# calad0i/da4ml

Hardware: AMD Instinct MI355X
Metric: CMVM solves/sec, 256x256 int8 matrix (higher is better)
Workload: dtype u32; 1 GPU; c3_256x256_int8_batch64_single_chain; matrix=256x256 int8 (default_rng(seed).integers(-128,128)), batch_per_gpu=64, parallelism=1 x independent-instance shard, no data-path collective

## Files before the change

### __graft_entry__.py

```python

import subprocess
import sys
from pathlib import Path

ROOT = Path(__file__).resolve().parent
if str(ROOT) not in sys.path:
    sys.path.insert(0, str(ROOT))


def build() -> None:
    subprocess.run(['make', '-C', str(ROOT / 'da4ml_amd' / 'csrc')], check=True)
    subprocess.run(['make', '-C', str(ROOT / 'oracle'), 'liboracle.so', 'ref'], check=True)
    subprocess.run(['make', '-C', str(ROOT / 'tests' / 'model')], check=True)
    subprocess.run(['make', '-C', str(ROOT / 'tests' / 'geometry')], check=True)
    subprocess.run(['make', '-C', str(ROOT / 'tests' / 'emu')], check=True)
    import da4ml_amd
    from da4ml_amd import _binary

    lib = _binary.lib()
    missing = [s for s in _binary.EXPORTS if not hasattr(lib, s)]
    assert not missing, f'libda4ml_hip.so lacks {missing}'


def smoke() -> None:
    import numpy as np

    from da4ml_amd import _binary
    from oracle.oracle import Oracle

    assert _binary.device_count() >= 1, 'smoke() needs a HIP device'
    k = np.random.default_rng(0).integers(-8, 8, (16, 16)).astype(np.float32)
    got = _binary.solve(k, adder_size=1, carry_size=-1)
    want = Oracle('port').solve(k, adder_size=1, carry_size=-1)
    assert got == want, 'HIP solve differs from the CPU oracle'
    assert np.all(got.kernel == k)
    print(f'smoke ok: 16x16 int4 cost={got.cost} adders={got.n_adders} latency={got.latency}')


if __name__ == '__main__':
    build()
    if len(sys.argv) > 1 and sys.argv[1] == 'smoke':
        smoke()
```

### da4ml_amd/csrc/cmvm_core.h

```cpp
#pragma once

#include <stdint.h>
#include <string.h>

#if defined(__HIPCC__)
#include <hip/hip_runtime.h>
#define DA_HD __host__ __device__ __forceinline__
#else
#define DA_HD inline
#endif

namespace da {

enum Method : int { M_MC = 0, M_MC_DC = 1, M_MC_PDC = 2, M_WMC = 3, M_WMC_DC = 4, M_WMC_PDC = 5, M_DUMMY = 6 };

enum ChainError : int {
    E_OK = 0,
    E_ROW_CAPACITY = 1,
    E_TABLE_CAPACITY = 2,
    E_LIST_CAPACITY = 3,
    E_FLOAT_DOMAIN = 4,
    E_COUNT_OVERFLOW = 5,
    E_REMOTE_ERROR = 6,
};

struct RowInfo {
    float lo, hi, step, lat;
};

DA_HD uint32_t f2u(float f) {
    uint32_t u;
    memcpy(&u, &f, 4);
    return u;
}
DA_HD float u2f(uint32_t u) {
    float f;
    memcpy(&f, &u, 4);
    return f;
}
DA_HD int popc32(uint32_t x) {
#if defined(__HIP_DEVICE_COMPILE__)
    return __popc(x);
#else
    return __builtin_popcount(x);
#endif
}
DA_HD int ctz32(uint32_t x) {
#if defined(__HIP_DEVICE_COMPILE__)
    return __ffs((int)x) - 1;
#else
    return __builtin_ctz(x);
#endif
}

template <class Cell> struct CellOps;
template <> struct CellOps<uint32_t> {
    static constexpr int HALF = 16;
    static DA_HD uint32_t plus(uint32_t c) { return c & 0xFFFFu; }
    static DA_HD uint32_t minus(uint32_t c) { return c >> 16; }
    static DA_HD uint32_t make(uint32_t p, uint32_t m) { return p | (m << 16); }
};
template <> struct CellOps<uint64_t> {
    static constexpr int HALF = 32;
    static DA_HD uint32_t plus(uint64_t c) { return (uint32_t)c; }
    static DA_HD uint32_t minus(uint64_t c) { return (uint32_t)(c >> 32); }
    static DA_HD uint64_t make(uint32_t p, uint32_t m) { return (uint64_t)p | ((uint64_t)m << 32); }
};

DA_HD int key_count(int n_bits) { return 2 * (2 * n_bits - 1); }
DA_HD int key_index(int shift, int sub, int n_bits) { return sub * (2 * n_bits - 1) + shift + (n_bits - 1); }
DA_HD void key_decode(int idx, int n_bits, int &shift, int &sub) {
    int w = 2 * n_bits - 1;
    sub = idx >= w;
    shift = idx - sub * w - (n_bits - 1);
}

DA_HD uint32_t take_from(uint32_t x, int s) { return s >= 0 ? (s >= 32 ? 0u : x >> s) : (-s >= 32 ? 0u : x << (-s)); }
DA_HD uint32_t move_by(uint32_t x, int s) { return take_from(x, -s); }

DA_HD void naf_masks(int32_t x, uint32_t &plus, uint32_t &minus) {
    uint32_t a = x < 0 ? (uint32_t)(-(int64_t)x) : (uint32_t)x;
    uint64_t x3 = (uint64_t)a * 3u;
    uint32_t pos = (uint32_t)((x3 & ~(uint64_t)a) >> 1);
    uint32_t neg = (uint32_t)((~x3 & (uint64_t)a) >> 1);
    plus = x < 0 ? neg : pos;
    minus = x < 0 ? pos : neg;
}
DA_HD int naf_weight(int32_t x) {
    uint32_t a = x < 0 ? (uint32_t)(-(int64_t)x) : (uint32_t)x;
    uint64_t x3 = (uint64_t)a * 3u;
    uint64_t d = (x3 ^ (uint64_t)a) >> 1;
    return popc32((uint32_t)d) + popc32((uint32_t)(d >> 32));
}
DA_HD int csd_width(uint32_t max_abs) {
    uint64_t t = 3ull * (max_abs ? max_abs : 1u);
    int n = 1;
    while ((1ull << (n + 1)) < t) ++n;
    return n;
}
DA_HD int lsb_loc(float x) {
    if (x == 0.0f) return 127;
    uint32_t b = f2u(x);
    int e = (int)((b >> 23) & 0xFF);
    uint32_t m = (b & 0x7FFFFFu) + (1u << 23);
    return (int)(int8_t)(e + ctz32(m) - 150);
}
DA_HD int iceil_log2(float x) {
    uint32_t b = f2u(x);
    int e = (int)((b >> 23) & 0xFF);
    return (int)(int8_t)(e - 127 + ((b & 0x7FFFFFu) != 0));
}
DA_HD float pow2f(int s) { return u2f((uint32_t)(s + 127) << 23); }

template <class Cell, class F> DA_HD void for_pairs_cross(Cell lo, Cell hi, int n_bits, F &&f) {
    using O = CellOps<Cell>;
    uint32_t lp = O::plus(lo), lm = O::minus(lo), hp = O::plus(hi), hm = O::minus(hi);
    uint32_t la = lp | lm, ha = hp | hm;
    while (la) {
        int p = ctz32(la);
        la &= la - 1;
        int sl = (lm >> p) & 1;
        uint32_t h = ha;
        while (h) {
            int q = ctz32(h);
            h &= h - 1;
            int sh = (hm >> q) & 1;
            f(key_index(q - p, sl ^ sh, n_bits));
        }
    }
}
template <class Cell, class F> DA_HD void for_pairs_self(Cell c, int n_bits, F &&f) {
    using O = CellOps<Cell>;
    uint32_t cp = O::plus(c), cm = O::minus(c);
    uint32_t all = cp | cm;
    uint32_t hi = all;
    while (hi) {
        int a = ctz32(hi);
        hi &= hi - 1;
        int sa = (cm >> a) & 1;
        uint32_t lo = all & ((1u << a) - 1u);
        while (lo) {
            int b = ctz32(lo);
            lo &= lo - 1;
            int sb = (cm >> b) & 1;
            f(key_index(b - a, sa ^ sb, n_bits));
        }
    }
}
template <class Cell, class F> DA_HD void for_pairs_part(Cell part, Cell y, bool x_is_lo, int n_bits, F &&f) {
    if (x_is_lo)
        for_pairs_cross<Cell>(part, y, n_bits, f);
    else
        for_pairs_cross<Cell>(y, part, n_bits, f);
}

template <class Cell> DA_HD void substitute_column(Cell a, Cell b, bool same_row, int shift, int sub, Cell &ma, Cell &mb) {
    using O = CellOps<Cell>;
    uint32_t ap = O::plus(a), am = O::minus(a);
    if (!same_row) {
        uint32_t bp = O::plus(b), bm = O::minus(b);
        uint32_t map = ap & take_from(sub ? bm : bp, shift);
        uint32_t mam = am & take_from(sub ? bp : bm, shift);
        uint32_t tp = move_by(map, shift), tm = move_by(mam, shift);
        ma = O::make(map, mam);
        mb = sub ? O::make(tm, tp) : O::make(tp, tm);
        return;
    }
    int rel = -shift;
    uint32_t avp = ap, avm = am, map = 0, mam = 0, mbp = 0, mbm = 0;
    for (int p = 0; p + rel < O::HALF; ++p) {
        uint32_t bit_lo = 1u << p, bit_hi = 1u << (p + rel);
        uint32_t all = avp | avm;
        if (!(all & bit_lo) || !(all & bit_hi)) continue;
        int s_lo = (avm & bit_lo) != 0, s_hi = (avm & bit_hi) != 0;
        if ((s_lo ^ s_hi) != sub) continue;
        avp &= ~(bit_lo | bit_hi);
        avm &= ~(bit_lo | bit_hi);
        if (s_hi)
            mam |= bit_hi;
        else
            map |= bit_hi;
        if (s_lo)
            mbm |= bit_lo;
        else
            mbp |= bit_lo;
    }
    ma = O::make(map, mam);
    mb = O::make(mbp, mbm);
}

DA_HD int n_overlap(const RowInfo &a, const RowInfo &b) {
    float hi0 = a.hi + a.step, hi1 = b.hi + b.step;
    float st = a.step > b.step ? a.step : b.step;
    int8_t f = (int8_t)(-iceil_log2(st));
    float m0 = __builtin_fabsf(a.lo) < __builtin_fabsf(hi0) ? __builtin_fabsf(hi0) : __builtin_fabsf(a.lo);
    float m1 = __builtin_fabsf(b.lo) < __builtin_fabsf(hi1) ? __builtin_fabsf(hi1) : __builtin_fabsf(b.lo);
    int8_t i_low = (int8_t)iceil_log2(m1 < m0 ? m1 : m0);
    int8_t k = (a.lo < 0 || b.lo < 0) ? 1 : 0;
    return (int)(int8_t)(k + i_low + f);
}

DA_HD uint32_t float_rank(float s) {
    if (s != s) return 0;
    if (s == 0.0f) s = 0.0f;
    uint32_t u = f2u(s == 0.0f ? 0.0f : s);
    return (u & 0x80000000u) ? ~u : (u | 0x80000000u);
}

DA_HD uint32_t entry_rank(uint32_t count, int ov, float dl, int method) {
    if (count < 2) return 0;
    switch (method) {
    case M_MC: return count + 1;
    case M_WMC: {
#if defined(__HIP_DEVICE_COMPILE__)
        if (count <= 0xFFFFu) {
            const int32_t s32 = (int32_t)count * ov;
            return s32 >= 0 ? (uint32_t)s32 + 1 : 0;
        }
#endif
        int64_t s = (int64_t)count * ov;
        return s >= 0 ? (uint32_t)s + 1 : 0;
    }
    case M_MC_DC:
    case M_MC_PDC: {
#if defined(__HIP_DEVICE_COMPILE__)
        float s = __fsub_rn((float)count, __fmul_rn(1e9f, dl));
#else
// ... 136 lines not shown
```

### da4ml_amd/csrc/cmvm_engine.hip

```cpp

#include <hip/hip_runtime.h>

#include <algorithm>
#include <atomic>
#include <chrono>
#include <cmath>
#include <cstdio>
#include <cstdlib>
#include <cstring>
#include <memory>
#include <mutex>
#include <numeric>
#include <stdexcept>
#include <string>
#include <thread>
#include <vector>

#include "cmvm_core.h"
#include "cmvm_geometry.h"
#include "cmvm_gpu.h"
#include "cmvm_host.h"

namespace da {
namespace gpu {
// ... 1927 lines not shown
            }
        }
        (void)w;
    }
    if (c.rword && part == 1) {
        const int nl = (int)gq->l_n[(gq->iter - 1) & 1];
        const CandEntry *ll = &gq->l_list[(gq->iter - 1) & 1][0];
        const uint32_t *colbits = gq->colbits;
        const int cbw = gq->cb_words;
        for (int e = (wave_id() + 2) % UPD_WAVES; e < nl; e += UPD_WAVES) {
            const unsigned long long tw = ll[e].tie;
            const uint32_t i0 = (uint32_t)((tw >> 7) & 0xFFFFFFu), i1 = (uint32_t)(tw >> 31);
            const uint32_t r = (i0 == A || i0 == B) ? i1 : i0;
            int hit = 0;
            for (int k = lane; k < u.m; k += WAVE) hit |= (int)((colbits[(size_t)u.mcol[k] * cbw + (r >> 5)] >> (r & 31)) & 1u);
            if (!__any(hit) && lane == 0) fold_entry(c, (uint32_t)ll[e].rank, tw);
        }
    }
}

template <class Cell, int NWV, bool STATS>
__device__ __forceinline__ void update_body(ChainDev *gq, bool in_range, int block_y, int grid_y) {
    constexpr int NTHR = NWV * WAVE;
    const UpdStep<Cell> u = load_upd_step<Cell>(gq);
    if (!in_range || u.done) return;
    if (block_y >= grid_y - 2) {
        special_pairs<Cell>(gq, u, block_y - (grid_y - 2));
        return;
    }
    grid_y -= 2;
    if (block_y * (NWV * QN) >= u.n_partners) return;
    extern __shared__ __attribute__((aligned(16))) unsigned char smem[];
    const int tid = threadIdx.x, lane = lane_id(), wid = wave_id();
    UpdLds<Cell> s;
    s.carve(smem, smem + align16(UpdLds<Cell>::table_bytes(u.c.n_out)) + (size_t)wid * UpdLds<Cell>::wave_bytes(u.c.Kpad), u.c.n_out);
    const int total_waves = grid_y * NWV, gw = block_y * NWV + wid;
    const unsigned long long ref0 = gw * QN + (lane >> QG_LOG2) < u.n_partners ? u.plist[gw * QN + (lane >> QG_LOG2)] : 0ull;
    const RowInfo rnew = load_row(u.c.rows, u.Nw);
    __shared__ unsigned int s_stat[3];
    if constexpr (STATS)
        if (tid < 3) s_stat[tid] = 0;
    copy_handoff<Cell>(u, s, tid, NTHR);
    __syncthreads();
    unsigned int found = 0, inserts = 0, deletes = 0;
    update_partners<Cell, STATS>(gq, u, s, gw * QN, total_waves * QN, u.n_partners, ref0, rnew, found, inserts, deletes);
    if constexpr (!STATS) return;
    if (lane == 0 && (found | inserts | deletes)) {
        if (found) atomicAdd(&s_stat[0], found);
        if (inserts) atomicAdd(&s_stat[1], inserts);
        if (deletes) atomicAdd(&s_stat[2], deletes);
    }
    __syncthreads();
    if (tid == 0) {
        if (s_stat[0]) atomicAdd(&gq->st_found, (unsigned long long)s_stat[0]);
        if (s_stat[1]) atomicAdd(&gq->st_inserts, (unsigned long long)s_stat[1]);
        if (s_stat[1] != s_stat[2]) atomicAdd(&gq->n_live, s_stat[1] - s_stat[2]);
    }
}
template <class Cell, bool STATS>
__global__ void __launch_bounds__(UPD_THREADS, DA_UPD_OCC) __attribute__((amdgpu_num_sgpr(DA_UPD_SGPRS))) k_iter_update(ChainDev *chains, int n_chains) {
#ifdef DA_STEP_CLOCKS
    ChainDev *gk = &chains[(int)blockIdx.x < n_chains ? blockIdx.x : 0];
    const bool clk_on = (int)blockIdx.x < n_chains && !gk->done;
    const int clk_par = (gk->iter - 1) & 1;
    if (clk_on && threadIdx.x == 0) CLK_MARK(gk, clk_par, 2, true);
#endif
    update_body<Cell, UPD_WAVES, STATS>(&chains[(int)blockIdx.x < n_chains ? blockIdx.x : 0], (int)blockIdx.x < n_chains, (int)blockIdx.y, (int)gridDim.y);
#ifdef DA_STEP_CLOCKS
    __syncthreads();
    if (clk_on && threadIdx.x == 0) CLK_MARK(gk, clk_par, 3, false);
#endif
}


template <class Cell> __global__ void __launch_bounds__(256) k_cs_init_counts(ChainDev *g) {
    const Ctx c = make_ctx(g, 0);
    extern __shared__ __attribute__((aligned(16))) unsigned char smem[];
    uint32_t *cnt = reinterpret_cast<uint32_t *>(smem) + (size_t)wave_id() * c.Kpad;
    const long long n_in = g->n_in, n_pairs = n_in * (n_in + 1) / 2;
    const long long p = (long long)blockIdx.x * (blockDim.x / WAVE) + wave_id();
    if (p >= n_pairs) return;
    long long i1 = (long long)((sqrt(8.0 * (double)p + 1.0) - 1.0) * 0.5);
    while (i1 * (i1 + 1) / 2 > p) --i1;
    while ((i1 + 1) * (i1 + 2) / 2 <= p) ++i1;
    const uint32_t hi = (uint32_t)i1, lo = (uint32_t)(p - i1 * (i1 + 1) / 2);
    count_row_pair<Cell>(c, reinterpret_cast<const typename RowFmt<Cell>::Entry *>(g->rlist), lo, hi, cnt);
    for (int k = lane_id(); k < c.K; k += WAVE) g->cs_init[(size_t)p * c.K + k] = (int32_t)cnt[k];
}
template <class Cell> __global__ void __launch_bounds__(256) k_cs_init_table(ChainDev *g) {
    const Ctx c = make_ctx(g, 0);
    const long long n_in = g->n_in, n_pairs = n_in * (n_in + 1) / 2;
    const long long p = (long long)blockIdx.x * (blockDim.x / WAVE) + wave_id();
    if (p >= n_pairs) return;
    long long i1 = (long long)((sqrt(8.0 * (double)p + 1.0) - 1.0) * 0.5);
    while (i1 * (i1 + 1) / 2 > p) --i1;
    while ((i1 + 1) * (i1 + 2) / 2 <= p) ++i1;
    const uint32_t hi = (uint32_t)i1, lo = (uint32_t)(p - i1 * (i1 + 1) / 2);
    const int32_t *cnt = g->cs_init + (size_t)p * c.K;
    int f = 0;
    for (int k = lane_id(); k < c.K; k += WAVE) f |= cnt[k] >= 2;
    if (!__any(f)) return;
    if (c.method < 0) {
        if (lane_id() == 0) g->unknown_hit = 1;
        return;
    }
    table_insert(c, lo, hi, load_row(c.rows, lo), load_row(c.rows, hi), [&](int k) { return (uint32_t)cnt[k]; });
}

__global__ void __launch_bounds__(1024) k_cs_union(ChainDev *g, volatile int *report, int seq, int flag_words) {
    __shared__ int s_part[16], s_base[17];
    const int tid = threadIdx.x, lane = lane_id(), wid = wave_id();
    const int n_rows = (int)g->Nw;
    const int per = (n_rows + 1023) / 1024;
    const int r0 = min(tid * per, n_rows), r1 = min(r0 + per, n_rows);
    int mine = 0;
    for (int r = r0; r < r1; ++r) mine += ((g->cs_flags[r >> 2] >> (8 * (r & 3))) & 0xFF) != 0;
    int inc = mine;
    for (int o = 1; o < WAVE; o <<= 1) {
        int t = __shfl_up(inc, o);
        if (lane >= o) inc += t;
    }
    if (lane == WAVE - 1) s_part[wid] = inc;
    __syncthreads();
    if (tid == 0) {
        int run = 0;
        for (int w = 0; w < 16; ++w) {
            s_base[w] = run;
            run += s_part[w];
        }
        s_base[16] = run;
        g->cs_nuni = run;
        if (report) {
            report[1] = run;
            report[2] = g->cs_flags[flag_words];
            report[3] = g->cs_flags[flag_words + 1];
            report[4] = g->cs_flags[flag_words + 2];
            __threadfence_system();
            report[0] = seq;
        }
    }
    __syncthreads();
    int at = s_base[wid] + inc - mine;
    for (int r = r0; r < r1; ++r)
        if (((g->cs_flags[r >> 2] >> (8 * (r & 3))) & 0xFF) != 0) g->cs_uni[at++] = (uint32_t)r;
}

template <class Cell> __global__ void __launch_bounds__(256) k_cs_partial(ChainDev *g) {
    using F = RowFmt<Cell>;
    using Entry = typename F::Entry;
    const Ctx c = make_ctx(g, 0);
    const int m = g->m, nb = c.n_bits, n_out = c.n_out, K = c.K, Kpad = c.Kpad;
    extern __shared__ __attribute__((aligned(16))) unsigned char smem[];
    Cell *s_mA = reinterpret_cast<Cell *>(smem);
    Cell *s_mB = s_mA + n_out;
    uint32_t *s_cnt = reinterpret_cast<uint32_t *>(s_mB + n_out);
    uint16_t *s_cmap = reinterpret_cast<uint16_t *>(s_cnt + 4 * 3 * Kpad);
    const int tid = threadIdx.x, lane = lane_id(), wid = wave_id();
    for (int j = tid; j < n_out; j += 256) s_cmap[j] = 0;
    __syncthreads();
    for (int j = tid; j < m; j += 256) {
        s_cmap[g->mcol[j]] = (uint16_t)(j + 1);
        s_mA[j] = reinterpret_cast<const Cell *>(g->mA)[j];
        s_mB[j] = reinterpret_cast<const Cell *>(g->mB)[j];
    }
    __syncthreads();
    const int u = (int)blockIdx.x * 4 + wid;
    if (u >= g->cs_nuni) return;
    const uint32_t A = g->A, B = g->B, r = g->cs_uni[u];
    const bool same = A == B;
    uint32_t *dA = s_cnt + (size_t)wid * 3 * Kpad, *dB = dA + Kpad, *cN = dB + Kpad;
    for (int k = lane; k < 3 * Kpad; k += WAVE) dA[k] = 0;
    lds_fence();
    const da_u2 ref = g->rowoff[r];
    const Entry *row = reinterpret_cast<const Entry *>(g->rlist) + ref.x;
    for (int j = lane; j < (int)ref.y; j += WAVE) {
        const Entry en = row[j];
        const Cell x = F::cell(en);
        if (!x) continue;
        const int at = (int)s_cmap[F::col(en)];
        if (!at) continue;
        const Cell ma = s_mA[at - 1], mb = s_mB[at - 1];
        for_pairs_part<Cell>(ma, x, A < r, nb, [&](int k) { atomicAdd(&dA[k], 1u); });
        if (same)
            for_pairs_part<Cell>(mb, x, A < r, nb, [&](int k) { atomicAdd(&dA[k], 1u); });
        else
            for_pairs_part<Cell>(mb, x, B < r, nb, [&](int k) { atomicAdd(&dB[k], 1u); });
        for_pairs_cross<Cell>(x, ma, nb, [&](int k) { atomicAdd(&cN[k], 1u); });
    }
    lds_fence();
    int32_t *out = g->cs_slab + (size_t)(6 + 3 * u) * K;
    for (int k = lane; k < K; k += WAVE) {
        out[k] = (int32_t)dA[k];
        out[K + k] = (int32_t)dB[k];
        out[2 * K + k] = (int32_t)cN[k];
    }
}

template <class Cell> __global__ void __launch_bounds__(256) k_cs_apply(ChainDev *g) {
    Ctx c = make_ctx(g, 2 * g->iter - 1);
    c.rword = g->spec[(g->iter - 1) & 1].word;
    c.cn = &g->c_n[(g->iter - 1) & 1];
    c.cl = &g->c_list[(g->iter - 1) & 1][0];
    const int K = c.K;
    const int w = (int)blockIdx.x * 4 + wave_id();
    const uint32_t A = g->A, B = g->B, Nw = g->Nw;
    const bool same = A == B;
    if (w == 5 && c.rword) {
        const int nl = (int)g->l_n[(g->iter - 1) & 1];
        const CandEntry *ll = &g->l_list[(g->iter - 1) & 1][0];
        if (lane_id() == 0)
            for (int e = 0; e < nl; ++e) {
                const unsigned long long tw = ll[e].tie;
                const uint32_t i0 = (uint32_t)((tw >> 7) & 0xFFFFFFu), i1 = (uint32_t)(tw >> 31);
                const uint32_t r = (i0 == A || i0 == B) ? i1 : i0;
                if (((g->cs_flags[r >> 2] >> (8 * (r & 3))) & 0xFF) == 0) fold_entry(c, (uint32_t)ll[e].rank, tw);
            }
    }
    if (w < 6) {
        uint32_t lo = A, hi = A;
        bool active = true, existed = false;
        switch (w) {
        case 0: lo = A, hi = A, existed = true; break;
        case 1: lo = A, hi = B, existed = true, active = !same; break;
        case 2: lo = B, hi = B, existed = true, active = !same; break;
        case 3: lo = A, hi = Nw; break;
        case 4: lo = B, hi = Nw, active = !same; break;
        default: lo = Nw, hi = Nw; break;
        }
        if (!active) return;
        const int32_t *cnt = g->cs_slab + (size_t)w * K;
        const unsigned long long key = pack_pair(lo, hi);
        const int slot = existed ? table_find(c, key, hash_pair(lo, hi)) : -1;
        if (slot >= 0)
            table_update(c, slot, key, [&](int k, uint32_t) { return (uint32_t)cnt[k]; });
        else {
            int f = 0;
            for (int k = lane_id(); k < K; k += WAVE) f |= cnt[k] >= 2;
            if (__any(f)) table_insert(c, lo, hi, load_row(c.rows, lo), load_row(c.rows, hi), [&](int k) { return (uint32_t)cnt[k]; });
        }
        return;
    }
    const int u = w - 6;
    if (u >= g->cs_nuni) return;
    const uint32_t r = g->cs_uni[u];
    const int32_t *dA = g->cs_slab + (size_t)(6 + 3 * u) * K, *dB = dA + K, *cN = dB + K;
    {
        const uint32_t lo = min(A, r), hi = max(A, r);
        const int slot = table_find(c, pack_pair(lo, hi), hash_pair(lo, hi));
        if (slot >= 0) table_update(c, slot, pack_pair(lo, hi), [&](int k, uint32_t old) { return old - (uint32_t)dA[k]; });
    }
    if (!same) {
        const uint32_t lo = min(B, r), hi = max(B, r);
        const int slot = table_find(c, pack_pair(lo, hi), hash_pair(lo, hi));
        if (slot >= 0) table_update(c, slot, pack_pair(lo, hi), [&](int k, uint32_t old) { return old - (uint32_t)dB[k]; });
    }
    int f = 0;
    for (int k = lane_id(); k < K; k += WAVE) f |= cN[k] >= 2;
    if (__any(f)) table_insert(c, r, Nw, load_row(c.rows, r), load_row(c.rows, Nw), [&](int k) { return (uint32_t)cN[k]; });
    if (lane_id() == 0) atomicAdd(&g->st_partners, 1ull);
}

template <class Cell> __global__ void __launch_bounds__(256) k_extract(ChainDev *chains) {
    using O = CellOps<Cell>;
    using F = RowFmt<Cell>;
    ChainDev &ch = chains[blockIdx.y];
    int j = blockIdx.x * (blockDim.x / WAVE) + wave_id();
    if (j >= ch.n_out) return;
    const auto *rl = reinterpret_cast<const typename F::Entry *>(ch.rlist);
    int lane = lane_id(), len = ch.collen[j], out = 0;
    for (int base = 0; base < len; base += WAVE) {
        int e = base + lane;
        Cell c = 0;
        uint32_t r = 0;
        if (e < len) {
            const unsigned long long ref = ch.collist[(size_t)j * ch.lcap + e];
            r = ref_row(ref);
            const auto *row = rl + ref_off(ref);
            if ((int)r < ch.n_in)
                c = F::cell(row[j]);
            else {
                int lo = 0, hi = (int)ref_len(ref) - 1;
                while (lo < hi) {
                    int mid = (lo + hi) >> 1;
                    if (F::col(row[mid]) < (uint32_t)j)
                        lo = mid + 1;
                    else
                        hi = mid;
                }
                const auto en = row[lo];
                c = F::col(en) == (uint32_t)j ? F::cell(en) : (Cell)0;
            }
        }
        unsigned long long nz = __ballot(c != 0);
        if (c != 0) {
            size_t at = (size_t)j * ch.lcap + out + __popcll(nz & ((1ull << lane) - 1));
            ch.fin_row[at] = r;
            ch.fin_cell[at] = (unsigned long long)O::plus(c) | ((unsigned long long)O::minus(c) << 32);
        }
        out += __popcll(nz);
    }
    if (lane == 0) ch.fin_count[j] = (uint32_t)out;
}

__global__ void __launch_bounds__(256) k_pack(ChainDev *chains) {
    ChainDev &ch = chains[blockIdx.x];
    __shared__ uint32_t s_total;
    const int n_out = ch.n_out, tid = threadIdx.x, lane = lane_id(), nw = blockDim.x / WAVE;
    if (tid < WAVE) {
        uint32_t run = 0;
        for (int base = 0; base < n_out; base += WAVE) {
            int j = base + lane;
            uint32_t v = j < n_out ? ch.fin_count[j] : 0u, inc = v;
            for (int o = 1; o < WAVE; o <<= 1) {
                uint32_t t = (uint32_t)__shfl_up((int)inc, o);
                if (lane >= o) inc += t;
            }
            if (j < n_out) ch.fin_start[j] = run + inc - v;
            run += (uint32_t)__shfl((int)inc, WAVE - 1);
        }
        if (lane == 0) {
            ch.fin_start[n_out] = run;
            ch.pk_total = run;
            s_total = run;
        }
    }
    __syncthreads();
    if (s_total > (uint32_t)ch.pk_cap) {
        if (tid == 0) ch.error = E_LIST_CAPACITY;
        return;
    }
    for (int j = wave_id(); j < n_out; j += nw) {
        const uint32_t cnt = ch.fin_count[j], dst = ch.fin_start[j];
        const size_t src = (size_t)j * ch.lcap;
        for (uint32_t e = lane; e < cnt; e += WAVE) {
            ch.pk_row[dst + e] = ch.fin_row[src + e];
            ch.pk_cell[dst + e] = ch.fin_cell[src + e];
        }
    }
    for (int r = tid; r < ch.n_rows; r += blockDim.x) ch.pk_lat[r] = ch.rows[r].lat;
}

struct GatherPiece {
    const void *src;
    unsigned long long dst_off, bytes;
};
__global__ void __launch_bounds__(256) k_gather(const GatherPiece *pieces, unsigned char *dst) {
// ... 782 lines not shown
        o.stats.digits0 = d.prep_digits;
        o.stats.table_peak = d.live_peak;
        o.stats.scan_slots = (long long)d.st_rescans << d.gs_log2;
        o.stats.partners = (long long)d.st_partners;
        o.stats.matches = (long long)d.st_matches;
        for (int q = 0; q < 12; ++q) im.timings.phase_cycles[q] += (double)d.st_phase[q];
        for (int q = 0; q < 4; ++q) im.timings.search_cycles[q] += (double)d.st_qphase[q];
        im.timings.search_diag[0] += (double)d.st_qdiag[0], im.timings.search_diag[1] += (double)d.st_qdiag[1], im.timings.search_diag[2] += (double)d.st_qdiag[4];
        im.timings.search_diag[3] += (double)d.st_qdiag[5], im.timings.search_diag[4] = std::max(im.timings.search_diag[4], (double)d.st_qdiag[6]), im.timings.search_diag[5] += (double)d.st_qdiag[7], im.timings.search_diag[6] += (double)d.st_qdiag[8];
        im.timings.fast_steps += (long long)d.st_fast;
        im.timings.found += (long long)d.st_found;
        im.timings.inserts += (long long)d.st_inserts;
        im.timings.cell_reads += (long long)d.st_cells;
        im.timings.key_bytes += 2.0 * d.K * (double)(d.st_found + d.st_inserts);
        im.timings.cell_bytes += (geo[i].wide ? 8.0 : 4.0) * (double)d.st_cells;
        im.timings.iterations += d.iter;
        im.timings.rescans += (long long)d.st_rescans;
        im.timings.select_bytes += (double)d.st_sel_bytes + 32.0 * (double)d.n_groups * (double)d.iter + (double)d.st_rescans * ((double)(4u << d.gs_log2) + 24.0);
        im.timings.partners += (long long)d.st_partners;
        im.timings.table_bytes += (double)d.C * (8.0 + 4.0 + (double)(1 << d.pb_log2));
    }
    lap("extract + download + unpack");
    im.timings.loop_ms += loop_ms;
    im.timings.host_launch_ms += host_launch_ms;
    im.timings.lockstep_iters += launched_iters;
    im.timings.chains += n;
    im.timings.arena_bytes = std::max(im.timings.arena_bytes, (double)arena_bytes);
    im.timings.total_ms += std::chrono::duration<double, std::milli>(std::chrono::steady_clock::now() - t_begin).count();
    (void)max_n_in;
}

namespace {

class HipShardEngine : public ShardEngine {
  public:
    HipShardEngine(hipStream_t st, int device, const ChainJob &job, int c0, int c1, double table_scale, double row_scale)
        : st_(st), device_(device), job_(job), n_loc_(c1 - c0) {
        HIP_CHECK(hipSetDevice(device_));
        const size_t e = (size_t)job.n_in * job.n_out;
        const size_t kb = align_up(e * 4, 256), qb = align_up((size_t)job.n_in * 12, 256), lb = align_up((size_t)job.n_in * 4, 256);
        io_.get(2 * kb + qb + lb + align_up(job.n_in, 256) + align_up(job.n_out, 256) + 256);
        unsigned char *io = static_cast<unsigned char *>(io_.ptr);
        std::memset(&d_, 0, sizeof d_);
        d_.n_in = job.n_in;
        d_.n_out = n_loc_;
        d_.pn_out = job.n_out;
        d_.col0 = c0;
        d_.method = job.method;
        d_.adder_size = job.adder_size;
        d_.carry_size = job.carry_size;
        d_.kernel = reinterpret_cast<const float *>(io);
        d_.qints = reinterpret_cast<const float *>(io + kb);
        d_.lats = reinterpret_cast<const float *>(io + kb + qb);
        d_.xint = reinterpret_cast<int32_t *>(io + kb + qb + lb);
        d_.shift0 = reinterpret_cast<int8_t *>(io + 2 * kb + qb + lb);
        d_.shift1 = d_.shift0 + align_up(job.n_in, 256);
        HIP_CHECK(hipMemcpyAsync(io, job.kernel, e * 4, hipMemcpyHostToDevice, st_));
        HIP_CHECK(hipMemcpyAsync(io + kb, job.qints, (size_t)job.n_in * 12, hipMemcpyHostToDevice, st_));
        HIP_CHECK(hipMemcpyAsync(io + kb + qb, job.lats, (size_t)job.n_in * 4, hipMemcpyHostToDevice, st_));
        desc_.get(sizeof(ChainDev));
        dd_ = static_cast<ChainDev *>(desc_.ptr);
        push();
        hipLaunchKernelGGL(k_prepare, dim3(1), dim3(256), (size_t)job.n_out * 4, st_, dd_);
        HIP_CHECK(hipGetLastError());
        pull();
        Geometry &g = geo_;
        g.n_bits = d_.prep_nbits;
        if (g.n_bits > 30) throw std::runtime_error("kernel needs more than 30 CSD digits per entry; unsupported");
        g.wide = g.n_bits > 12 || n_loc_ > 256;
        if (job.adder_size >= 0 || job.carry_size >= 0) step_tab_.build(job.qints, job.n_in);
        g.n_mant = (int)step_tab_.mant.size();
        g.K = key_count(g.n_bits);
        g.Kpad = (g.K + 3) & ~3;
        g.pb_log2 = 5;
        while ((1 << g.pb_log2) < 16 + 2 * g.Kpad) ++g.pb_log2;
        const long long D0 = d_.prep_digits;
        const TableGeometry tg = table_geometry(job, d_.prep_pairs, D0, table_scale, row_scale, MAX_GROUPS);
        g.rcap = tg.rcap < (1 << REF_ROW_BITS) ? (int)tg.rcap : (1 << REF_ROW_BITS);
        g.lcap = job.n_in + d_.prep_maxdcol + 1;
        g.pk_cap = (int)std::min<long long>(D0 + 1, (long long)1 << 30);
        const long long rl_want = (long long)job.n_in * n_loc_ + D0 + n_loc_ + 64;
        if (rl_want >= (1ll << REF_OFF_BITS) || g.rcap >= (1 << REF_ROW_BITS) || n_loc_ >= (1 << REF_LEN_BITS))
            throw std::runtime_error("problem too large for the row-reference format");
        g.rl_cap = (uint32_t)rl_want;
        g.C = tg.C;
        g.gs_log2 = tg.gs_log2;
        g.n_groups = tg.n_groups;
        n_pairs_ = (long long)job.n_in * (job.n_in + 1) / 2;
        ChainJob local = job;
        local.n_out = n_loc_;
        ChainDev tmp;
        const size_t chain_bytes = carve_chain(nullptr, local, g, tmp);
        const size_t init_b = align_up((size_t)n_pairs_ * g.K * 4, 256), flag_b = align_up((((size_t)g.rcap + 3) / 4 + SHARD_TRAILER) * 4 + 64, 256),
                     uni_b = align_up((size_t)g.rcap * 4, 256), slab_b = align_up((size_t)(6 + 3 * (size_t)g.rcap) * g.K * 4, 256);
        const size_t need = chain_bytes + init_b + flag_b + uni_b + slab_b;
        {
            size_t free_b = 0, total_b = 0;
            HIP_CHECK(hipMemGetInfo(&free_b, &total_b));
            if (need > free_b)
                throw std::runtime_error("a column-sharded chain needs " + std::to_string(need >> 20) + " MiB of device memory (pair table of " +
                                         std::to_string(g.C) + " slots), " + std::to_string(free_b >> 20) + " MiB are free");
        }
        arena_.get(need);
        unsigned char *a = static_cast<unsigned char *>(arena_.ptr);
        carve_chain(a, local, g, d_);
        d_.cs_init = reinterpret_cast<int32_t *>(a + chain_bytes);
        d_.cs_flags = reinterpret_cast<int32_t *>(a + chain_bytes + init_b);
        d_.cs_uni = reinterpret_cast<uint32_t *>(a + chain_bytes + init_b + flag_b);
        d_.cs_slab = reinterpret_cast<int32_t *>(a + chain_bytes + init_b + flag_b + uni_b);
        d_.n_bits = g.n_bits;
        d_.K = g.K;
        d_.Kpad = g.Kpad;
        d_.rcap = g.rcap;
        d_.lcap = g.lcap;
        d_.gs_log2 = g.gs_log2;
        d_.n_groups = g.n_groups;
        d_.C = g.C;
        d_.cmask = g.C - 1;
        d_.pb_log2 = g.pb_log2;
        d_.rl_cap = g.rl_cap;
        d_.rl_used = (uint32_t)job.n_in * (uint32_t)n_loc_;
        d_.n_rows = job.n_in;
        d_.claim_words = claim_words_for(local_job(), g, sel2_lds_budget(device_, g.wide));
        HIP_CHECK(hipMemsetAsync(d_.stamp, 0, sizeof(uint32_t) * (size_t)g.rcap, st_));
        HIP_CHECK(hipMemsetAsync(d_.hkey, 0xFF, sizeof(unsigned long long) * (size_t)g.C, st_));
        HIP_CHECK(hipMemsetAsync(d_.hrank, 0, sizeof(uint32_t) * (size_t)g.C, st_));
        HIP_CHECK(hipMemsetAsync(d_.grec, 0, sizeof(GroupRec) * (size_t)g.n_groups, st_));
        d_.cb_words = (g.rcap + 31) / 32;
        HIP_CHECK(hipMemsetAsync(d_.colbits, 0, sizeof(uint32_t) * (size_t)n_loc_ * d_.cb_words, st_));
        {
            d_.n_step_mant = (int)step_tab_.mant.size();
            if (d_.n_step_mant) {
                HIP_CHECK(hipMemcpyAsync(const_cast<uint32_t *>(d_.step_mant), step_tab_.mant.data(), step_tab_.mant.size() * 4, hipMemcpyHostToDevice, st_));
                HIP_CHECK(hipMemcpyAsync(const_cast<float *>(d_.step_tab), step_tab_.tab.data(), step_tab_.tab.size() * 4, hipMemcpyHostToDevice, st_));
            }
        }
        push();
        report_ = static_cast<volatile int *>(report_buf_.get(64));
        for (int q = 0; q < 5; ++q) report_[q] = 0;
        d_done_ = static_cast<unsigned int *>(done_buf_.get(sizeof(unsigned int)));
        HIP_CHECK(hipMemsetAsync(d_done_, 0, sizeof(unsigned int), st_));
        dim3 colgrid((n_loc_ + 3) / 4, 1);
        if (!g.wide)
            hipLaunchKernelGGL(k_init_cells<uint32_t>, colgrid, dim3(256), 0, st_, dd_);
        else
            hipLaunchKernelGGL(k_init_cells<uint64_t>, colgrid, dim3(256), 0, st_, dd_);
        HIP_CHECK(hipGetLastError());
        sel_lds_ = align_up(sel2_fixed_lds(local_job(), g) + (size_t)d_.claim_words * 4, 16);
        if (sel_lds_ > sel2_lds_budget(device_, g.wide)) throw std::runtime_error("selection kernel needs more dynamic LDS than the device leaves beside its static arrays (n_out too large)");
        if (!g.wide)
            HIP_CHECK(hipFuncSetAttribute(reinterpret_cast<const void *>(&k_iter_select2<uint32_t, true>), hipFuncAttributeMaxDynamicSharedMemorySize, (int)sel_lds_));
        else
            HIP_CHECK(hipFuncSetAttribute(reinterpret_cast<const void *>(&k_iter_select2<uint64_t, true>), hipFuncAttributeMaxDynamicSharedMemorySize, (int)sel_lds_));
        part_lds_ = align_up(2 * (size_t)n_loc_ * (g.wide ? 8 : 4) + 4 * 3 * (size_t)g.Kpad * 4 + (size_t)n_loc_ * 2, 16);
        HIP_CHECK(hipStreamSynchronize(st_));
    }
    ~HipShardEngine() override { (void)hipSetDevice(device_); }
    bool on_device() const override { return true; }
    int n_keys() const override { return geo_.K; }
    int32_t *init_counts(int64_t &count) override {
        const dim3 grid((unsigned)((n_pairs_ + 3) / 4));
        if (!geo_.wide)
            hipLaunchKernelGGL(k_cs_init_counts<uint32_t>, grid, dim3(256), (size_t)4 * geo_.Kpad * 4, st_, dd_);
        else
            hipLaunchKernelGGL(k_cs_init_counts<uint64_t>, grid, dim3(256), (size_t)4 * geo_.Kpad * 4, st_, dd_);
        sync();
        count = n_pairs_ * geo_.K;
        return d_.cs_init;
    }
    void init_table() override {
        const dim3 grid((unsigned)((n_pairs_ + 3) / 4));
        if (!geo_.wide)
            hipLaunchKernelGGL(k_cs_init_table<uint32_t>, grid, dim3(256), 0, st_, dd_);
        else
            hipLaunchKernelGGL(k_cs_init_table<uint64_t>, grid, dim3(256), 0, st_, dd_);
        HIP_CHECK(hipGetLastError());
    }
    void set_stream_ordered(bool on) override { stream_ordered_ = on; }
    void select(int32_t *&flags, int64_t &fcount) override {
        fw_ = flag_words(job_.n_in + (int)steps_);
        if (!stopped_) {
            if (!geo_.wide)
                hipLaunchKernelGGL((k_iter_select2<uint32_t, true>), dim3(1, 2), dim3(SEL2_THREADS), sel_lds_, st_, dd_, 1, d_done_, (int)steps_);
            else
                hipLaunchKernelGGL((k_iter_select2<uint64_t, true>), dim3(1, 2), dim3(SEL2_THREADS), sel_lds_, st_, dd_, 1, d_done_, (int)steps_);
            HIP_CHECK(hipGetLastError());
        } else {
            const int32_t tr[SHARD_TRAILER] = {1, 0, 0};
            HIP_CHECK(hipMemsetAsync(d_.cs_flags, 0, (size_t)fw_ * 4, st_));
            HIP_CHECK(hipMemcpyAsync(d_.cs_flags + fw_, tr, sizeof tr, hipMemcpyHostToDevice, st_));
            sync();
        }
        if (!stream_ordered_) sync();
        flags = d_.cs_flags;
        fcount = fw_ + SHARD_TRAILER;
    }
    int32_t *partial(int64_t &scount, int32_t status[SHARD_TRAILER]) override {
        const int seq = ++report_seq_;
        hipLaunchKernelGGL(k_cs_union, dim3(1), dim3(1024), 0, st_, dd_, report_, seq, (int)fw_);
        HIP_CHECK(hipGetLastError());
        {
            unsigned polls = 0, tries = 0;
            while (__atomic_load_n(&report_[0], __ATOMIC_ACQUIRE) != seq) {
                if (++tries > (1u << 16)) {
                    sync();
                    if (__atomic_load_n(&report_[0], __ATOMIC_ACQUIRE) != seq) throw std::runtime_error("column-sharded chain: the device did not report the step's status");
                    break;
                }
                spin_wait_step(polls);
            }
        }
        const int nuni = report_[1];
        for (int q = 0; q < SHARD_TRAILER; ++q) trailer_[q] = report_[2 + q];
        for (int q = 0; q < SHARD_TRAILER; ++q) status[q] = trailer_[q];
        scount = 0;
        if (status[0] != 0) {
            stopped_ = true;
            return nullptr;
        }
        nuni_ = nuni;
        if (nuni > 0) {
            const dim3 grid((unsigned)((nuni + 3) / 4));
            if (!geo_.wide)
                hipLaunchKernelGGL(k_cs_partial<uint32_t>, grid, dim3(256), part_lds_, st_, dd_);
            else
                hipLaunchKernelGGL(k_cs_partial<uint64_t>, grid, dim3(256), part_lds_, st_, dd_);
        }
        if (!stream_ordered_) sync();
        scount = (int64_t)(6 + 3 * (int64_t)nuni) * geo_.K;
        return d_.cs_slab;
    }
    void apply() override {
        const dim3 grid((unsigned)((nuni_ + 6 + 3) / 4));
        if (!geo_.wide)
            hipLaunchKernelGGL(k_cs_apply<uint32_t>, grid, dim3(256), 0, st_, dd_);
        else
            hipLaunchKernelGGL(k_cs_apply<uint64_t>, grid, dim3(256), 0, st_, dd_);
        HIP_CHECK(hipGetLastError());
        ++steps_;
    }
    void finish(ChainOut &o) override {
        dim3 colgrid((n_loc_ + 3) / 4, 1);
        if (!geo_.wide)
            hipLaunchKernelGGL(k_extract<uint32_t>, colgrid, dim3(256), 0, st_, dd_);
        else
            hipLaunchKernelGGL(k_extract<uint64_t>, colgrid, dim3(256), 0, st_, dd_);
        hipLaunchKernelGGL(k_pack, dim3(1), dim3(256), 0, st_, dd_);
        pull();
        o = ChainOut{};
        o.error = d_.error;
        o.unknown_method_hit = d_.unknown_hit != 0;
        o.n_bits = d_.n_bits;
        const size_t iters = (size_t)d_.iter;
        o.shift0.resize(job_.n_in);
        o.shift1.resize(job_.n_out);
        o.picks.resize(iters * 4);
        o.row_lat.resize((size_t)d_.n_rows);
        o.col_start.resize((size_t)n_loc_ + 1);
        HIP_CHECK(hipMemcpyAsync(o.shift0.data(), d_.shift0, job_.n_in, hipMemcpyDeviceToHost, st_));
        HIP_CHECK(hipMemcpyAsync(o.shift1.data(), d_.shift1, job_.n_out, hipMemcpyDeviceToHost, st_));
        if (iters) HIP_CHECK(hipMemcpyAsync(o.picks.data(), d_.picks, iters * sizeof(int4), hipMemcpyDeviceToHost, st_));
        HIP_CHECK(hipMemcpyAsync(o.row_lat.data(), d_.pk_lat, (size_t)d_.n_rows * 4, hipMemcpyDeviceToHost, st_));
        HIP_CHECK(hipMemcpyAsync(o.col_start.data(), d_.fin_start, ((size_t)n_loc_ + 1) * 4, hipMemcpyDeviceToHost, st_));
        sync();
        const size_t total = o.col_start[n_loc_];
        o.dig_row.resize(total);
        std::vector<unsigned long long> cells(total);
        if (total) {
            HIP_CHECK(hipMemcpyAsync(o.dig_row.data(), d_.pk_row, total * 4, hipMemcpyDeviceToHost, st_));
            HIP_CHECK(hipMemcpyAsync(cells.data(), d_.pk_cell, total * 8, hipMemcpyDeviceToHost, st_));
            sync();
        }
        o.dig_cell.assign(cells.begin(), cells.end());
        o.stats.iterations = d_.iter;
        o.stats.digits0 = d_.prep_digits;
        o.stats.table_peak = d_.live_peak;
        o.stats.partners = (long long)d_.st_partners;
        o.stats.matches = (long long)d_.st_matches;
        o.stats.scan_slots = (long long)d_.st_rescans << d_.gs_log2;
    }

  private:
    ChainJob local_job() const {
        ChainJob j = job_;
        j.n_out = n_loc_;
        return j;
    }
    void sync() {
        HIP_CHECK(hipGetLastError());
        HIP_CHECK(hipStreamSynchronize(st_));
    }
    void push() { HIP_CHECK(hipMemcpyAsync(dd_, &d_, sizeof d_, hipMemcpyHostToDevice, st_)); }
    void pull() {
        HIP_CHECK(hipGetLastError());
        HIP_CHECK(hipMemcpyAsync(&d_, dd_, sizeof d_, hipMemcpyDeviceToHost, st_));
        HIP_CHECK(hipStreamSynchronize(st_));
    }
    hipStream_t st_;
    StepLog2Host step_tab_;
    int64_t fw_ = 0;
    long long steps_ = 0;
    bool stopped_ = false, stream_ordered_ = false;
    int32_t trailer_[SHARD_TRAILER] = {0, 0, 0};
    int device_;
    ChainJob job_;
    int n_loc_;
    ChainDev d_;
// ... 121 lines not shown
```

Baseline: 112.0 solves/s.

## Derive partial pair-loss counts from cross histogram instead of separate atomics

The partial count-update kernel no longer accumulates separate dA/dB histograms with LDS atomics. It builds only the cross-pair histogram cN and derives the loss counts for A and B by remapping key indices through a new loss_source helper, using the picked shift and sub. This removes two of the three atomic passes per row entry and shrinks LDS per block. The cost is reliance on an algebraic identity between the histograms, which must hold exactly for correctness.

```diff
diff --git a/__graft_entry__.py b/__graft_entry__.py
--- a/__graft_entry__.py
+++ b/__graft_entry__.py
@@ -13,6 +13,7 @@
     subprocess.run(['make', '-C', str(ROOT / 'oracle'), 'liboracle.so', 'ref'], check=True)
     subprocess.run(['make', '-C', str(ROOT / 'tests' / 'model')], check=True)
     subprocess.run(['make', '-C', str(ROOT / 'tests' / 'geometry')], check=True)
+    subprocess.run(['make', '-C', str(ROOT / 'tests' / 'pairmap')], check=True)
     subprocess.run(['make', '-C', str(ROOT / 'tests' / 'emu')], check=True)
     import da4ml_amd
     from da4ml_amd import _binary
diff --git a/da4ml_amd/csrc/cmvm_core.h b/da4ml_amd/csrc/cmvm_core.h
--- a/da4ml_amd/csrc/cmvm_core.h
+++ b/da4ml_amd/csrc/cmvm_core.h
@@ -73,6 +73,15 @@
     int w = 2 * n_bits - 1;
     sub = idx >= w;
     shift = idx - sub * w - (n_bits - 1);
+}
+
+DA_HD int loss_source(int k, int n_bits, bool mirror, int shift, int sub) {
+    const int w = 2 * n_bits - 1;
+    if (k < 0 || k >= 2 * w) return -1;
+    const int sg = k >= w, dt = k - sg * w - (n_bits - 1);
+    const int d = (mirror ? -dt : dt) - shift;
+    if (d <= -n_bits || d >= n_bits) return -1;
+    return (sg ^ sub) * w + d + (n_bits - 1);
 }
 
 DA_HD uint32_t take_from(uint32_t x, int s) { return s >= 0 ? (s >= 32 ? 0u : x >> s) : (-s >= 32 ? 0u : x << (-s)); }
diff --git a/da4ml_amd/csrc/cmvm_engine.hip b/da4ml_amd/csrc/cmvm_engine.hip
--- a/da4ml_amd/csrc/cmvm_engine.hip
+++ b/da4ml_amd/csrc/cmvm_engine.hip
@@ -2103,24 +2103,22 @@
     const int m = g->m, nb = c.n_bits, n_out = c.n_out, K = c.K, Kpad = c.Kpad;
     extern __shared__ __attribute__((aligned(16))) unsigned char smem[];
     Cell *s_mA = reinterpret_cast<Cell *>(smem);
-    Cell *s_mB = s_mA + n_out;
-    uint32_t *s_cnt = reinterpret_cast<uint32_t *>(s_mB + n_out);
-    uint16_t *s_cmap = reinterpret_cast<uint16_t *>(s_cnt + 4 * 3 * Kpad);
+    uint32_t *s_cnt = reinterpret_cast<uint32_t *>(s_mA + n_out);
+    uint16_t *s_cmap = reinterpret_cast<uint16_t *>(s_cnt + 4 * Kpad);
     const int tid = threadIdx.x, lane = lane_id(), wid = wave_id();
     for (int j = tid; j < n_out; j += 256) s_cmap[j] = 0;
     __syncthreads();
     for (int j = tid; j < m; j += 256) {
         s_cmap[g->mcol[j]] = (uint16_t)(j + 1);
         s_mA[j] = reinterpret_cast<const Cell *>(g->mA)[j];
-        s_mB[j] = reinterpret_cast<const Cell *>(g->mB)[j];
     }
     __syncthreads();
     const int u = (int)blockIdx.x * 4 + wid;
     if (u >= g->cs_nuni) return;
     const uint32_t A = g->A, B = g->B, r = g->cs_uni[u];
     const bool same = A == B;
-    uint32_t *dA = s_cnt + (size_t)wid * 3 * Kpad, *dB = dA + Kpad, *cN = dB + Kpad;
-    for (int k = lane; k < 3 * Kpad; k += WAVE) dA[k] = 0;
+    uint32_t *cN = s_cnt + (size_t)wid * Kpad;
+    for (int k = lane; k < Kpad; k += WAVE) cN[k] = 0;
     lds_fence();
     const da_u2 ref = g->rowoff[r];
     const Entry *row = reinterpret_cast<const Entry *>(g->rlist) + ref.x;
@@ -2130,19 +2128,19 @@
         if (!x) continue;
         const int at = (int)s_cmap[F::col(en)];
         if (!at) continue;
-        const Cell ma = s_mA[at - 1], mb = s_mB[at - 1];
-        for_pairs_part<Cell>(ma, x, A < r, nb, [&](int k) { atomicAdd(&dA[k], 1u); });
-        if (same)
-            for_pairs_part<Cell>(mb, x, A < r, nb, [&](int k) { atomicAdd(&dA[k], 1u); });
-        else
-            for_pairs_part<Cell>(mb, x, B < r, nb, [&](int k) { atomicAdd(&dB[k], 1u); });
-        for_pairs_cross<Cell>(x, ma, nb, [&](int k) { atomicAdd(&cN[k], 1u); });
+        for_pairs_cross<Cell>(x, s_mA[at - 1], nb, [&](int k) { atomicAdd(&cN[k], 1u); });
     }
     lds_fence();
     int32_t *out = g->cs_slab + (size_t)(6 + 3 * u) * K;
+    const int pk_shift = g->pk_shift, pk_sub = g->pk_sub;
+    auto lost = [&](int k, bool mir, int sh, int sb) {
+        const int s_ = loss_source(k, nb, mir, sh, sb);
+        return s_ < 0 ? 0u : cN[s_];
+    };
     for (int k = lane; k < K; k += WAVE) {
-        out[k] = (int32_t)dA[k];
-        out[K + k] = (int32_t)dB[k];
+        const uint32_t viaB = lost(k, B < r, pk_shift, pk_sub);
+        out[k] = (int32_t)(lost(k, A < r, 0, 0) + (same ? viaB : 0u));
+        out[K + k] = (int32_t)(same ? 0u : viaB);
         out[2 * K + k] = (int32_t)cN[k];
     }
 }
@@ -3231,7 +3229,7 @@
             HIP_CHECK(hipFuncSetAttribute(reinterpret_cast<const void *>(&k_iter_select2<uint32_t, true>), hipFuncAttributeMaxDynamicSharedMemorySize, (int)sel_lds_));
         else
             HIP_CHECK(hipFuncSetAttribute(reinterpret_cast<const void *>(&k_iter_select2<uint64_t, true>), hipFuncAttributeMaxDynamicSharedMemorySize, (int)sel_lds_));
-        part_lds_ = align_up(2 * (size_t)n_loc_ * (g.wide ? 8 : 4) + 4 * 3 * (size_t)g.Kpad * 4 + (size_t)n_loc_ * 2, 16);
+        part_lds_ = align_up((size_t)n_loc_ * (g.wide ? 8 : 4) + 4 * (size_t)g.Kpad * 4 + (size_t)n_loc_ * 2, 16);
         HIP_CHECK(hipStreamSynchronize(st_));
     }
     ~HipShardEngine() override { (void)hipSetDevice(device_); }
```

Result: no change. 111.9 solves/s (median of 2 runs) (-0.1%).
